# leochlon/aecf

Measured on AMD Instinct MI355X. Metric: fused samples/sec (fwd+bwd), higher is better.
Workload: dtype bf16; 1 GPU; c2: [B=65536 per GPU, M=3, d=512, 8 heads] mask_prob=0.15 train-mode curriculum masking, fwd+bwd; global_batch=65536, parallelism=dp1, world_size=1

## Files before the change

### aecf_amd/csrc/aecf_capi.hip

```cpp
#include <math.h>
#include <stdio.h>
#include <stdint.h>


#include "../../include/aecf_hip.h"
#include "aecf_kernels.h"

using namespace aecf;

namespace {

inline size_t align_up(size_t v, size_t a = 256) { return (v + a - 1) / a * a; }
inline int esize(int dtype) { return dtype == AECF_F32 ? 4 : 2; }
inline bool ws_frag_shape(int dtype, int E) { return dtype == AECF_BF16 && (E == 256 || E == 512 || E == 768 || E == 1024); }

struct FwdWs {
    size_t qs, a_f32, a_hi, a_lo, obuf, wv_frag, wo_frag, total;
};
FwdWs fwd_layout(const aecf_pool_desc* d) {
    FwdWs w;
    const size_t E = d->embed_dim, es = esize(d->dtype);
    size_t off = 0;
    w.qs = off;    off = align_up(off + E * 4);
    w.a_f32 = off; off = align_up(off + HPAD * E * 4);
// ... 399 lines not shown
    const BwdWs L = bwd_layout(d, hilo);
    if (a->workspace_bytes < L.total) return AECF_ERR_WORKSPACE;
    char* ws = (char*)a->workspace;
    const int E = d->embed_dim, H = d->num_heads, M = d->modalities, hd = E / H, es = esize(d->dtype);
    const int64_t B = d->batch;
    const PrepWs& P = L.prep;
    char* pb = a->saved_prep ? (char*)const_cast<void*>(a->saved_prep) : ws;
    float* qs = (float*)(pb + P.qs);
    float* a_f32 = (float*)(pb + P.a_f32);
    void* wvt = pb + P.wvt;
    void* wot = pb + P.wot;
    void* dobuf = do_ready ? const_cast<void*>(do_ready) : (void*)(ws + L.dobuf);
    float* dsbuf = (float*)(ws + L.dsbuf);
    float* u = (float*)(ws + L.u);
    const float scale = sqrtf(1.0f / (float)hd);
    const char* w_v = (const char*)a->w_in + (size_t)2 * E * E * es;

    void** ev = a->stage_events;
    mark(ev, 0, s);
    const bool frag = ws_frag_shape(d->dtype, E);
    FragJobs fj;
    if (!a->saved_prep) {
        if (frag) {
            fj.n = 2;
            fj.src[0] = w_v;      fj.dst[0] = pb + P.wvt_frag; fj.transposed[0] = 1;
            fj.src[1] = a->w_out; fj.dst[1] = pb + P.wot_frag; fj.transposed[1] = 1;
        }
        launch_prep_all(d->dtype, a->w_in, a->b_in, a->query, scale, qs, a_f32, pb + P.a_hi, pb + P.a_lo, w_v, wvt, a->w_out,
                        wot, E, H, fj, s);
    }
    mark(ev, 1, s);

    GemmNtArgs g;
    g.a = a->dy; g.w = wot; g.bias = nullptr; g.c = dobuf; g.probs = nullptr; g.R = B; g.N = E; g.K = E; g.lda = E;
    g.M = 1; g.H = H; g.hd = hd; g.pooled = 0; g.out_f32 = 0; g.v_out = nullptr;
    if (frag) g.w_frag = pb + P.wot_frag;
    if (hilo) g.c_lo = ws + L.do_lo;
    if (!do_ready) launch_gemm_nt(d->dtype, g, s);
    mark(ev, 2, s);

    GemmTnArgs t1;
    t1.lhs = a->dy; t1.rhs = a->saved_o; t1.probs = nullptr; t1.dsbuf = nullptr; t1.out = (float*)(ws + L.slab_o);
    t1.colsum = (float*)(ws + L.cs_o); t1.u = nullptr; t1.B = B; t1.M = 1; t1.E = E; t1.H = H; t1.hd = hd;
    t1.Ej = 0; t1.splits = L.splits; t1.rows_per_split = L.rows_per_split; t1.pooled = 0;
    t1.u_splits = 0; t1.u_rows_per_split = 0;
    if (hilo) {
        t1.rhs_lo = a->saved_o_lo;
        launch_gemm_tn_hilo(t1, s);
    } else {
        launch_gemm_tn(d->dtype, t1, s);
    }
    const int gt = a->grad_dtype == AECF_BF16 ? GRAD_BF16 : (a->grad_dtype == AECF_F16 ? GRAD_F16 : GRAD_F32);
    mark(ev, 3, s);

    BwdGArgs g2;
    g2.x = a->x; g2.dobuf = dobuf; g2.wvt = wvt; g2.probs = a->saved_probs; g2.d_attn_w = a->d_attn_w;
    g2.d_entropy = a->d_entropy; g2.attn_w = a->attn_w; g2.dsbuf = dsbuf; g2.a_f32 = a_f32; g2.dx = a->dx;
    g2.B = B; g2.M = M; g2.E = E; g2.H = H; g2.hd = hd; g2.log_M = (float)log((double)M);
    if (frag) g2.wvt_frag = pb + P.wvt_frag;
    int dsu_chunks = 0;
    if (hilo) g2.do_lo = ws + L.do_lo;
    const bool dsu = d->dtype == AECF_BF16 && dsu_ws_chunks(g2) > 0 && dsu_ws_chunks(g2) <= L.u_splits_cap &&
                     (!hilo || dsu_ws_takes_lo(g2));
    if (dsu)
        dsu_chunks = launch_dsu_ws(g2, (float*)(ws + L.u_slab), s);
    else if (!(!hilo && a->saved_v && launch_dscore_v(d->dtype, g2, a->saved_v, s)))
        launch_bwd_g(d->dtype, g2, false, s);
    mark(ev, 4, s);

    GemmTnArgs t2;
    t2.lhs = dobuf; t2.rhs = a->x; t2.probs = a->saved_probs; t2.dsbuf = dsbuf; t2.out = (float*)(ws + L.slab_v);
    t2.colsum = (float*)(ws + L.cs_v); t2.u = (float*)(ws + L.u_slab); t2.B = B; t2.M = M; t2.E = E; t2.H = H;
    t2.hd = hd; t2.Ej = 0; t2.splits = L.splits; t2.rows_per_split = L.rows_per_split; t2.pooled = 1;
    t2.u_splits = L.u_splits; t2.u_rows_per_split = L.u_rows_per_split;
    if (!dsu_chunks) {
        t2.parts = 2;
        launch_gemm_tn(d->dtype, t2, s);
    }
    mark(ev, 5, s);
    const bool dx_last = a->param_grads_event != nullptr;
    constexpr int DX_RESERVE_CUS = 16;
    if (dx_last) g2.cu_budget = 256 - DX_RESERVE_CUS;
    bool u_reduced = false;
    if (!dx_last) { g2.u_slab_in = (const float*)(ws + L.u_slab); g2.u_out = u; g2.u_nslab = dsu_chunks ? dsu_chunks : L.u_splits; }
    auto run_dx = [&]() {
        if (d->dtype == AECF_BF16 && launch_dx_ws(g2, s)) { u_reduced = g2.u_slab_in != nullptr; return; }
        launch_bwd_g(d->dtype, g2, true, s);
    };
// ... 633 lines not shown
```

### aecf_amd/csrc/aecf_gemm_ws.hip

```cpp
#include <stdlib.h>

#include "aecf_kernels.h"
#include "aecf_tile.h"

namespace aecf {

namespace {

enum { WS_PLAIN = 0, WS_VPROJ = 1, WS_VFLAT = 2 };

constexpr int WS_PF = 3, VPROJ_PF = 3, DX_PF = 3;

constexpr int ws_plain_bufs(int, int) { return 2; }

template <int KT, int NROWS, int KEYDIV>
__device__ __forceinline__ void ws_dma_rows(const char* __restrict__ src, unsigned int ld_bytes, int rows_valid, char* lds) {
    constexpr int CPR = 4 * KT;
    constexpr int TOTAL = NROWS * CPR;
    constexpr int NI = (TOTAL + 511) / 512;
    static_assert(TOTAL % 64 == 0, "whole wave-instructions");
    const int wbase = __builtin_amdgcn_readfirstlane((int)(threadIdx.x & ~63u));
#pragma unroll
    for (int i = 0; i < NI; ++i) {
        if (wbase + 512 * i < TOTAL) {
// ... 528 lines not shown
                for (int c = 0; c < CT; ++c) asm volatile("" : "+v"(acc[m][c]));
            __builtin_amdgcn_sched_barrier(0);
#pragma unroll
            for (int c = 0; c < CT; ++c) Pc[c] = Pn[c];
        }

        asm volatile("s_waitcnt vmcnt(0)" ::: "memory");
        if (o0 + 16 < o_end) park_stage(cur ^ 1);
        const int64_t b = o0 + r16;
        if (b < o_end) {
#pragma unroll
            for (int m = 0; m < M_; ++m) {
                float v[NV];
#pragma unroll
                for (int c = 0; c < CT; ++c)
#pragma unroll
                    for (int r = 0; r < 4; ++r) v[4 * c + r] = acc[m][c][r];
                store_cols<CT>(reinterpret_cast<unsigned short*>(p.dx) + (b * M_ + m) * E + ncol0 + NV * lg, v);
            }
        }
    }
}

template <int KT, int HK, int M_, bool HILO>
__global__ __launch_bounds__(512, 2) void dsu_ws_kernel(BwdGArgs p, float* __restrict__ u_slab, int rows_per_block, int nchunk) {
    using X = Tr<BF16>;
    constexpr int KJ = 8;
    constexpr int E = 32 * KT, JB = 32 * KJ, NCT = KT / 4;
    constexpr int HBL = KJ / HK;
    constexpr int ROWX = 2 * E, ROWD = 2 * JB;
    constexpr int XROWS = 16 * M_;
    constexpr int KU = (XROWS + 31) / 32;
    constexpr int ZROWS = (32 * KU - XROWS) > 0 ? 1 : 0;
    constexpr int PSTR = HBL * M_ * 16;
    constexpr int DSROW = 72;
    constexpr int XT = XROWS * ROWX, DT = 16 * ROWD;
    constexpr int NPART = 8;
    extern __shared__ __attribute__((aligned(16))) char smem[];
    char* xb = smem;
    char* zp = smem + 2 * XT;
    char* db = zp + ZROWS * ROWX;
    char* dbl = db + 2 * DT;
    float* part = reinterpret_cast<float*>(db + (HILO ? 4 : 2) * DT);
    unsigned short* dsh = reinterpret_cast<unsigned short*>(reinterpret_cast<char*>(part) + NPART * PSTR * 4);
    unsigned short* dsl = dsh + 16 * DSROW;

    const int lane = lane_id(), r16 = lane & 15, lg = lane >> 4;
    const int w = __builtin_amdgcn_readfirstlane(wave_id());
    const int H = p.H;
    unsigned int chunk_u, group_u;
    if (!xcd_tile(blockIdx.x, (unsigned)nchunk, (unsigned)(E / JB), chunk_u, group_u)) return;
    const int jbase = (int)group_u * JB, hbase = jbase / (32 * HK);
    const int ncol0 = 16 * NCT * w;
    const int64_t o_beg = (int64_t)chunk_u * rows_per_block;
    const int64_t o_end = (o_beg + rows_per_block) < p.B ? (o_beg + rows_per_block) : p.B;
    if (o_beg >= o_end) return;

    const char* dsrc = reinterpret_cast<const char*>(p.dobuf) + (int64_t)jbase * 2;
    const char* xsrc = reinterpret_cast<const char*>(p.x);
    const char* dlsrc = HILO ? reinterpret_cast<const char*>(p.do_lo) + (int64_t)jbase * 2 : dsrc;
    auto issue = [&](int64_t o0, int buf) {
        const int ov = (int)((o_end - o0) < 16 ? (o_end - o0) : 16);
        ws_dma_rows_asm<KT, 16 * M_, M_>(xsrc + o0 * M_ * (int64_t)ROWX, (unsigned)ROWX, ov * M_, xb + buf * XT);
        ws_dma_rows_asm<KJ, 16, 1>(dsrc + o0 * (int64_t)ROWX, (unsigned)ROWX, ov, db + buf * DT);
        if (HILO) ws_dma_rows_asm<KJ, 16, 1>(dlsrc + o0 * (int64_t)ROWX, (unsigned)ROWX, ov, dbl + buf * DT);
    };
    for (int i = threadIdx.x; i < ZROWS * ROWX / 16; i += 512) reinterpret_cast<u32x4*>(zp)[i] = u32x4{0u, 0u, 0u, 0u};
    for (int i = threadIdx.x; i < 2 * 16 * DSROW / 2; i += 512) reinterpret_cast<unsigned int*>(dsh)[i] = 0u;
    issue(o_beg, 0);

    const unsigned short* wsrc = reinterpret_cast<const unsigned short*>(p.wvt);
    u32x4 wreg[KJ][NCT];
    static_assert(NCT % 2 == 0, "tile pairs");
#pragma unroll
    for (int ct = 0; ct < NCT; ++ct) {
        const int krow = ncol0 + 32 * (ct >> 1) + 8 * (r16 >> 2) + 4 * (ct & 1) + (r16 & 3);
        const unsigned short* wr = wsrc + (int64_t)krow * E + jbase + 8 * lg;
#pragma unroll
        for (int ks = 0; ks < KJ; ++ks) wreg[ks][ct] = *reinterpret_cast<const u32x4*>(wr + 32 * ks);
    }
    int daddr[4];
#pragma unroll
    for (int v = 0; v < 4; ++v) daddr[v] = r16 * ROWD + ((((4 * v) + lg) ^ r16) << 4);
    const int xaddr0 = r16 * M_ * ROWX + ((((ncol0 >> 3) + lg) ^ r16) << 4);
    const int q = r16 >> 2, pp = r16 & 3;
    int ua[KU][2];
    bool uz[KU][2];
#pragma unroll
    for (int ks = 0; ks < KU; ++ks) {
#pragma unroll
        for (int hh = 0; hh < 2; ++hh) {
            const int D = 4 * ks + 2 * hh + (lg >> 1);
            uz[ks][hh] = D >= 2 * M_;
            const int m = D >> 1, b = 2 * (4 * (lg & 1) + q) + (D & 1);
            const int key = uz[ks][hh] ? 0 : b;
            const int ch = ((ncol0 >> 3) + (pp >> 1)) ^ key;
            ua[ks][hh] = (uz[ks][hh] ? (int)(zp - smem) : (b * M_ + m) * ROWX) + (ch << 4) + 8 * (pp & 1);
        }
    }
    auto kslot = [&](int b, int m) -> int {
        const int D = 2 * m + (b & 1), j = b >> 1;
        return 32 * (D >> 2) + 8 * (2 * (D & 1) + (j >> 2)) + 4 * ((D >> 1) & 1) + (j & 3);
    };

    const int ds_s = lane & 15, ds_hh = w, ds_m = lg;
    const float invH = 1.0f / (float)H;
    auto load_stats = [&](int64_t o0, float& pmv, float& dwb) {
        int64_t b = o0 + ds_s;
        b = b < o_end ? b : o_end - 1;
        const float* pp_ = p.probs + (b * H + hbase + ds_hh) * M_ + (ds_m < M_ ? ds_m : 0);
        const float* dw_ = p.d_attn_w ? p.d_attn_w + b * M_ + (ds_m < M_ ? ds_m : 0) : pp_;
        if (w < HBL) {
            asm volatile("global_load_dword %0, %1, off" : "=v"(pmv) : "v"(pp_) : "memory");
            asm volatile("global_load_dword %0, %1, off" : "=v"(dwb) : "v"(dw_) : "memory");
        }
    };

    f32x4 uacc[NCT];
#pragma unroll
    for (int ct = 0; ct < NCT; ++ct) uacc[ct] = f32x4{0.f, 0.f, 0.f, 0.f};
    float pmv = 0.f, dwb = 0.f, pmv_n = 0.f, dwb_n = 0.f;
#pragma unroll
    for (int ks = 0; ks < KJ; ++ks)
#pragma unroll
        for (int ct = 0; ct < NCT; ++ct) asm volatile("" : "+v"(wreg[ks][ct]));
    load_stats(o_beg, pmv, dwb);

    asm volatile("s_waitcnt vmcnt(0)" ::: "memory");
    asm volatile("s_waitcnt lgkmcnt(0)" ::: "memory");
    int cur = 0;
    for (int64_t o0 = o_beg; o0 < o_end; o0 += 16, cur ^= 1) {
        __builtin_amdgcn_s_barrier();
        if (o0 + 16 < o_end) {
            issue(o0 + 16, cur ^ 1);
            load_stats(o0 + 16, pmv_n, dwb_n);
        }
        const char* tb = db + cur * DT;
        constexpr int HG = HBL % 2 == 0 ? 2 : 1;
        int xa[NCT];
#pragma unroll
        for (int ct = 0; ct < NCT; ++ct) xa[ct] = cur * XT + (xaddr0 ^ (64 * (ct >> 1)));
        float* pw = part + w * PSTR + r16;
#pragma unroll
        for (int h0 = 0; h0 < HBL; h0 += HG) {
            f32x4 P[HG][NCT];
#pragma unroll
            for (int g = 0; g < HG; ++g) {
#pragma unroll
                for (int ct = 0; ct < NCT; ++ct) P[g][ct] = f32x4{0.f, 0.f, 0.f, 0.f};
#pragma unroll
                for (int kl = 0; kl < HK; ++kl) {
                    const int ks = (h0 + g) * HK + kl;
                    const u32x4 bf = *reinterpret_cast<const u32x4*>(tb + daddr[ks & 3] + (ks >> 2) * 256);
#pragma unroll
                    for (int ct = 0; ct < NCT; ++ct) P[g][ct] = X::mma(wreg[ks][ct], bf, P[g][ct]);
                    if (HILO) {
                        const u32x4 bl = *reinterpret_cast<const u32x4*>(dbl + cur * DT + daddr[ks & 3] + (ks >> 2) * 256);
#pragma unroll
                        for (int ct = 0; ct < NCT; ++ct) P[g][ct] = X::mma(wreg[ks][ct], bl, P[g][ct]);
                    }
                }
            }
#pragma unroll
            for (int m = 0; m < M_; ++m) {
                float a[HG];
#pragma unroll
                for (int g = 0; g < HG; ++g) a[g] = 0.f;
#pragma unroll
                for (int c2 = 0; c2 < NCT / 2; ++c2) {
                    const u32x4 xv = *reinterpret_cast<const u32x4*>(xb + xa[2 * c2] + m * ROWX);
                    float xf[8];
#pragma unroll
                    for (int i = 0; i < 4; ++i) {
                        xf[2 * i] = __uint_as_float(xv[i] << 16);
                        xf[2 * i + 1] = __uint_as_float(xv[i] & 0xffff0000u);
                    }
#pragma unroll
                    for (int g = 0; g < HG; ++g)
#pragma unroll
                        for (int i = 0; i < 8; ++i) a[g] = fmaf(P[g][2 * c2 + (i >> 2)][i & 3], xf[i], a[g]);
                }
                const unsigned int u0 = __float_as_uint(a[0]), u1 = __float_as_uint(a[HG - 1]);
                const auto r1 = __builtin_amdgcn_permlane16_swap(u0, u1, false, false);
                const unsigned int us = __float_as_uint(__uint_as_float(r1[0]) + __uint_as_float(r1[1]));
                const auto r2 = __builtin_amdgcn_permlane32_swap(us, us, false, false);
                pw[((h0 + (HG == 2 ? (lg & 1) : 0)) * M_ + m) * 16] = __uint_as_float(r2[0]) + __uint_as_float(r2[1]);
            }
        }
        asm volatile("s_waitcnt lgkmcnt(0)" ::: "memory");
        __builtin_amdgcn_s_barrier();
        asm volatile("" : "+v"(pmv), "+v"(dwb));
        if (w < HBL) {
            float da = 0.f;
            if (ds_m < M_) {
                const float* pr = part + (ds_hh * M_ + ds_m) * 16 + ds_s;
#pragma unroll
                for (int i = 0; i < NPART; ++i) da += pr[i * PSTR];
            }
            float dw = p.d_attn_w ? dwb : 0.f;
            if (p.d_entropy && ds_m < M_) {
                int64_t be = o0 + ds_s;
                be = be < o_end ? be : o_end - 1;
                float hsum = 0.f;
#pragma unroll
                for (int m = 0; m < M_; ++m) hsum -= xlogx(p.attn_w[be * M_ + m]);
                const bool live = (hsum >= 0.f) && (hsum <= p.log_M);
                dw += live ? -(logf(p.attn_w[be * M_ + ds_m]) + 1.0f) * p.d_entropy[be] : 0.f;
            }
            const float dp = da + dw * invH;
            const float dot = reduce_lg((ds_m < M_) ? pmv * dp : 0.f);
            const int64_t b = o0 + ds_s;
            if (ds_m < M_) {
                const float d = (b < o_end) ? pmv * (dp - dot) : 0.f;
                if (b < o_end) p.dsbuf[(b * H + hbase + ds_hh) * M_ + ds_m] = d;
                const unsigned short hi = X::from_f32(d);
                dsh[ds_hh * DSROW + kslot(ds_s, ds_m)] = hi;
                dsl[ds_hh * DSROW + kslot(ds_s, ds_m)] = X::from_f32(d - X::to_f32(hi));
            }
        }
        asm volatile("s_waitcnt lgkmcnt(0)" ::: "memory");
        __builtin_amdgcn_s_barrier();
#pragma unroll
        for (int ks = 0; ks < KU; ++ks) {
            const u32x4 bh = *reinterpret_cast<const u32x4*>(reinterpret_cast<const char*>(dsh) + (r16 * DSROW + 32 * ks + 8 * lg) * 2);
            const u32x4 bl = *reinterpret_cast<const u32x4*>(reinterpret_cast<const char*>(dsl) + (r16 * DSROW + 32 * ks + 8 * lg) * 2);
#pragma unroll
            for (int ct = 0; ct < NCT; ++ct) {
                const u32x4 af = tr_frag16(smem, (uz[ks][0] ? 0 : cur * XT) + (ua[ks][0] ^ (32 * ct)),
                                           (uz[ks][1] ? 0 : cur * XT) + (ua[ks][1] ^ (32 * ct)));
                uacc[ct] = X::mma(af, bh, uacc[ct]);
                uacc[ct] = X::mma(af, bl, uacc[ct]);
            }
        }
        asm volatile("s_waitcnt vmcnt(0)" ::: "memory");
        asm volatile("" : "+v"(pmv_n), "+v"(dwb_n));
        pmv = pmv_n; dwb = dwb_n;
    }
    if (r16 < HBL) {
#pragma unroll
        for (int ct = 0; ct < NCT; ++ct)
            *reinterpret_cast<f32x4*>(u_slab + ((int64_t)chunk_u * H + hbase + r16) * E + ncol0 + 16 * ct + 4 * lg) = uacc[ct];
    }
}


static size_t dsu_ws_smem(int E, int M, int hd, bool lo) {
    constexpr int JB = 256;
    const int xrows = 16 * M, zrows = (32 * ((xrows + 31) / 32) - xrows) > 0 ? 1 : 0, hbl = JB / hd;
    return (size_t)(2 * xrows + zrows) * 2 * E + (size_t)(lo ? 4 : 2) * 16 * 2 * JB + (size_t)8 * (16 * hbl * M) * 4 +
           (size_t)2 * 16 * 72 * 2;
}

template <int KT, int HK, int M_>
int launch_dsu_t(const BwdGArgs& a, float* u_slab, hipStream_t s) {
    constexpr int E = 32 * KT, JB = 256;
    const bool hilo = a.do_lo && dsu_ws_takes_lo(a);
    const size_t smem = dsu_ws_smem(E, M_, a.hd, hilo);
    const int groups = E / JB;
    int64_t chunks = 256 / groups;
    if (chunks < 1) chunks = 1;
    int64_t rpb = (a.B + chunks - 1) / chunks;
    rpb = (rpb + 15) / 16 * 16;
    const int64_t nchunk = (a.B + rpb - 1) / rpb;
    dim3 grid(xcd_grid((unsigned)nchunk, (unsigned)groups)), block(512);
    if constexpr (!(E == 512 && M_ == 4)) {
        if (hilo) {
            auto kern = dsu_ws_kernel<KT, HK, M_, true>;
            (void)hipFuncSetAttribute(reinterpret_cast<const void*>(kern), hipFuncAttributeMaxDynamicSharedMemorySize, (int)smem);
            kern<<<grid, block, smem, s>>>(a, u_slab, (int)rpb, (int)nchunk);
            return (int)nchunk;
        }
    }
    auto kern = dsu_ws_kernel<KT, HK, M_, false>;
    (void)hipFuncSetAttribute(reinterpret_cast<const void*>(kern), hipFuncAttributeMaxDynamicSharedMemorySize, (int)smem);
    kern<<<grid, block, smem, s>>>(a, u_slab, (int)rpb, (int)nchunk);
    return (int)nchunk;
}

template <int KT, int HK, int M_>
void launch_dx2(const BwdGArgs& a, hipStream_t s) {
    constexpr int K = 32 * KT;
    constexpr int CT = KT <= 16 ? 2 : 1;
    constexpr int KX = (3 * (KT / HK) + 31) / 32;
    const size_t smem = (size_t)2 * 16 * 2 * K + (size_t)2 * 16 * (((KT / HK) * M_) | 1) * sizeof(float) + (size_t)2 * 16 * M_ * (64 * KX + 16);
    const int groups = a.E / (128 * CT);
    int64_t chunks = (a.cu_budget > 0 ? a.cu_budget : 256) / groups;
    if (chunks < 1) chunks = 1;
    int64_t rpb = (a.B + chunks - 1) / chunks;
    rpb = (rpb + 15) / 16 * 16;
    const int64_t nchunk = (a.B + rpb - 1) / rpb;
    dim3 grid(xcd_grid((unsigned)nchunk, (unsigned)groups)), block(512);
    auto kern = dx_ws2_kernel<KT, HK, M_, CT>;
    if (smem > 64 * 1024)
        (void)hipFuncSetAttribute(reinterpret_cast<const void*>(kern), hipFuncAttributeMaxDynamicSharedMemorySize, (int)smem);
    kern<<<grid, block, smem, s>>>(a, (int)rpb, (int)nchunk);
}

template <int KT, int HK>
void launch_dx2_m(const BwdGArgs& a, hipStream_t s) {
    switch (a.M) {
        case 1: launch_dx2<KT, HK, 1>(a, s); break;
// ... 301 lines not shown
    return a.lda == a.K;
}

void launch_gemm_ws(const GemmNtArgs& a, hipStream_t s) {
    if (ws_vproj_flat(a)) {
        GemmNtArgs f = a;
        f.R = a.R * a.M;
        f.lda = a.K;
        launch_kt<WS_VFLAT, 4, false>(f, s);
        return;
    }
    if (a.pooled & 1) {
        switch (a.M) {
            case 1: if (a.g_ahi) launch_kt<WS_VPROJ, 1, true>(a, s); else launch_kt<WS_VPROJ, 1, false>(a, s); break;
            case 2: if (a.g_ahi) launch_kt<WS_VPROJ, 2, true>(a, s); else launch_kt<WS_VPROJ, 2, false>(a, s); break;
            case 3: if (a.g_ahi) launch_kt<WS_VPROJ, 3, true>(a, s); else launch_kt<WS_VPROJ, 3, false>(a, s); break;
            default: launch_kt<WS_VPROJ, 4, false>(a, s); break;
        }
    } else {
        launch_kt<WS_PLAIN, 1, false>(a, s);
    }
}

int dsu_ws_chunks(const BwdGArgs& a) {
    if (a.M < 1 || a.M > 4 || a.hd % 32 != 0 || a.E != a.H * a.hd) return 0;
    if (a.E != 256 && a.E != 512) return 0;
    const int jb = 256;
    if (jb % a.hd != 0) return 0;
    const int hk = a.hd / 32;
    if (hk != 1 && hk != 2 && hk != 4 && hk != 8) return 0;
    if (dsu_ws_smem(a.E, a.M, a.hd, false) > 160 * 1024) return 0;
    const int groups = a.E / jb;
    int64_t chunks = 256 / groups;
    int64_t rpb = (a.B + chunks - 1) / chunks;
    rpb = (rpb + 15) / 16 * 16;
    return (int)((a.B + rpb - 1) / rpb);
}

bool dsu_ws_takes_lo(const BwdGArgs& a) {
    return dsu_ws_chunks(a) > 0 && dsu_ws_smem(a.E, a.M, a.hd, true) <= 160 * 1024;
}

template <int KT, int HK>
static int launch_dsu_m(const BwdGArgs& a, float* u_slab, hipStream_t s) {
    switch (a.M) {
        case 1: return launch_dsu_t<KT, HK, 1>(a, u_slab, s);
        case 2: return launch_dsu_t<KT, HK, 2>(a, u_slab, s);
        case 3: return launch_dsu_t<KT, HK, 3>(a, u_slab, s);
        default: return launch_dsu_t<KT, HK, 4>(a, u_slab, s);
    }
}

int launch_dsu_ws(const BwdGArgs& a, float* u_slab, hipStream_t s) {
    if (dsu_ws_chunks(a) == 0) return 0;
    const int hk = a.hd / 32;
#define DSU_CASE(KT_)                                                   \
    switch (hk) {                                                       \
        case 1: return launch_dsu_m<KT_, 1>(a, u_slab, s);              \
        case 2: return launch_dsu_m<KT_, 2>(a, u_slab, s);              \
        case 4: return launch_dsu_m<KT_, 4>(a, u_slab, s);              \
        default: return launch_dsu_m<KT_, 8>(a, u_slab, s);             \
    }
    if (a.E == 256) { DSU_CASE(8) }
    DSU_CASE(16)
#undef DSU_CASE
}

bool launch_dx_ws(const BwdGArgs& a, hipStream_t s) {
    if (a.M < 1 || a.M > 4) return false;
    if (a.hd % 32 != 0 || a.E != a.H * a.hd || 16 * a.H * a.M > 1024) return false;
    switch (a.E) {
        case 256: return launch_dx2_hk<8>(a, s);
        case 512: return launch_dx2_hk<16>(a, s);
        case 768: return launch_dx2_hk<24>(a, s);
        case 1024: return launch_dx2_hk<32>(a, s);
        default: return false;
    }
}

}
```

### aecf_amd/csrc/aecf_kernels.h

```cpp
#pragma once
#include <hip/hip_runtime.h>
#include <stdint.h>

#include "aecf_common.h"

namespace aecf {

constexpr int HPAD = 16;

void launch_prep_qs(int dtype, const void* w_in, const void* b_in, const void* query, float* qs, int E, float scale,
                    hipStream_t s);
void launch_prep_amat(int dtype, const void* w_in, const float* qs, float* a_f32, void* a_hi, void* a_lo, int E, int H,
                      hipStream_t s);
void launch_transpose(int dtype, const void* src, void* dst, int E, hipStream_t s);
struct FragJobs {
    int n = 0;
    const void* src[4] = {nullptr, nullptr, nullptr, nullptr};
    void* dst[4] = {nullptr, nullptr, nullptr, nullptr};
    int transposed[4] = {0, 0, 0, 0};
};
void launch_prep_all(int dtype, const void* w_in, const void* b_in, const void* query, float scale, float* qs, float* a_f32,
                     void* a_hi, void* a_lo, const void* t_src0, void* t_dst0, const void* t_src1, void* t_dst1, int E,
                     int H, const FragJobs& fj, hipStream_t s);

// ... 57 lines not shown
    const void* dobuf;
    const void* wvt;
    const float* probs;
    const float* d_attn_w;
    const float* d_entropy;
    const float* attn_w;
    float* dsbuf;
    const float* a_f32;
    void* dx;
    int64_t B;
    int M, E, H, hd;
    float log_M;
    const void* wvt_frag = nullptr;
    int cu_budget = 0;
    const float* u_slab_in = nullptr;
    float* u_out = nullptr;
    int u_nslab = 0;
    const void* do_lo = nullptr;
};
void launch_bwd_g(int dtype, const BwdGArgs& a, bool dx, hipStream_t s);
bool launch_dscore_v(int dtype, const BwdGArgs& a, const void* saved_v, hipStream_t s);
bool launch_dx_ws(const BwdGArgs& a, hipStream_t s);
int dsu_ws_chunks(const BwdGArgs& a);
int launch_dsu_ws(const BwdGArgs& a, float* u_slab, hipStream_t s);
bool dsu_ws_takes_lo(const BwdGArgs& a);

struct GemmTnArgs {
    const void* lhs;
    const void* rhs;
    const float* probs;
    const float* dsbuf;
    float* out;
    float* colsum;
    float* u;
    int64_t B;
    int M, E, H, hd;
    int Ej;
    int splits;
    int64_t rows_per_split;
    int u_splits;
    int64_t u_rows_per_split;
    int pooled;
    int parts = 0;
    DqpJob dq;
    const void* lhs_lo = nullptr;
    const void* rhs_lo = nullptr;
};
// ... 123 lines not shown
```

Before: 123.1 million samples/s.

## Reassociate dscore backward to project x through Wv instead of dO through WvT

Replaces the fused dscore+u kernel with a new one that computes v = x·Wv per modality (Wv held in registers, loaded from a newly prepared non-transposed fragment copy) and dots it with dO directly. The old path staged dO tiles into LDS and multiplied by WvT to get P before dotting with x. The change removes dO LDS staging and the per-head P accumulators, cutting LDS footprint and MMA work per row block. In exchange it needs an extra weight-fragment prep job, and the associativity change alters rounding.

```diff
diff --git a/aecf_amd/csrc/aecf_capi.hip b/aecf_amd/csrc/aecf_capi.hip
--- a/aecf_amd/csrc/aecf_capi.hip
+++ b/aecf_amd/csrc/aecf_capi.hip
@@ -445,9 +445,10 @@
     FragJobs fj;
     if (!a->saved_prep) {
         if (frag) {
-            fj.n = 2;
+            fj.n = 3;
             fj.src[0] = w_v;      fj.dst[0] = pb + P.wvt_frag; fj.transposed[0] = 1;
             fj.src[1] = a->w_out; fj.dst[1] = pb + P.wot_frag; fj.transposed[1] = 1;
+            fj.src[2] = w_v;      fj.dst[2] = pb + P.wv_frag;  fj.transposed[2] = 0;
         }
         launch_prep_all(d->dtype, a->w_in, a->b_in, a->query, scale, qs, a_f32, pb + P.a_hi, pb + P.a_lo, w_v, wvt, a->w_out,
                         wot, E, H, fj, s);
@@ -486,7 +487,7 @@
     const bool dsu = d->dtype == AECF_BF16 && dsu_ws_chunks(g2) > 0 && dsu_ws_chunks(g2) <= L.u_splits_cap &&
                      (!hilo || dsu_ws_takes_lo(g2));
     if (dsu)
-        dsu_chunks = launch_dsu_ws(g2, (float*)(ws + L.u_slab), s);
+        dsu_chunks = launch_dsu_ws(g2, w_v, frag ? pb + P.wv_frag : nullptr, (float*)(ws + L.u_slab), s);
     else if (!(!hilo && a->saved_v && launch_dscore_v(d->dtype, g2, a->saved_v, s)))
         launch_bwd_g(d->dtype, g2, false, s);
     mark(ev, 4, s);
diff --git a/aecf_amd/csrc/aecf_dsv_ws.hip b/aecf_amd/csrc/aecf_dsv_ws.hip
--- /dev/null
+++ b/aecf_amd/csrc/aecf_dsv_ws.hip
@@ -0,0 +1,314 @@
+#include "aecf_kernels.h"
+#include "aecf_tile.h"
+
+namespace aecf {
+
+namespace {
+
+constexpr int DSV_PF = 3;
+
+template <int KT, int HK, int M_, bool HILO>
+__global__ __launch_bounds__(512, 2) void dsv_ws_kernel(BwdGArgs p, const void* __restrict__ wv, const void* __restrict__ wv_frag,
+                                                         float* __restrict__ u_slab, int rows_per_block, int nchunk) {
+    using X = Tr<BF16>;
+    constexpr int E = 32 * KT, JB = 256, NCT = KT / 4;
+    constexpr int HBL = 8 / HK;
+    constexpr int ROWX = 2 * E;
+    constexpr int XROWS = 16 * M_;
+    constexpr int KU = (XROWS + 31) / 32;
+    constexpr int ZROWS = (32 * KU - XROWS) > 0 ? 1 : 0;
+    constexpr int PSTR = M_ * 16;
+    constexpr int DSROW = 72;
+    constexpr int XT = XROWS * ROWX;
+    extern __shared__ __attribute__((aligned(16))) char smem[];
+    char* xb = smem;
+    char* zp = smem + 2 * XT;
+    float* part = reinterpret_cast<float*>(zp + ZROWS * ROWX);
+    unsigned short* dsh = reinterpret_cast<unsigned short*>(reinterpret_cast<char*>(part) + 8 * PSTR * 4);
+    unsigned short* dsl = dsh + 16 * DSROW;
+
+    const int lane = lane_id(), r16 = lane & 15, lg = lane >> 4;
+    const int w = __builtin_amdgcn_readfirstlane(wave_id());
+    const int H = p.H;
+    unsigned int chunk_u, group_u;
+    if (!xcd_tile(blockIdx.x, (unsigned)nchunk, (unsigned)(E / JB), chunk_u, group_u)) return;
+    const int jbase = (int)group_u * JB, hbase = jbase / (32 * HK);
+    const int jcol0 = jbase + 32 * w;
+    const int ncol0 = 16 * NCT * w;
+    const int64_t o_beg = (int64_t)chunk_u * rows_per_block;
+    const int64_t o_end = (o_beg + rows_per_block) < p.B ? (o_beg + rows_per_block) : p.B;
+    if (o_beg >= o_end) return;
+
+    const char* xsrc = reinterpret_cast<const char*>(p.x);
+    auto issue = [&](int64_t o0, int buf) {
+        const int ov = (int)((o_end - o0) < 16 ? (o_end - o0) : 16);
+        ws_dma_rows_asm<KT, 16 * M_, M_>(xsrc + o0 * M_ * (int64_t)ROWX, (unsigned)ROWX, ov * M_, xb + buf * XT);
+    };
+    for (int i = threadIdx.x; i < ZROWS * ROWX / 16; i += 512) reinterpret_cast<u32x4*>(zp)[i] = u32x4{0u, 0u, 0u, 0u};
+    for (int i = threadIdx.x; i < 2 * 16 * DSROW / 2; i += 512) reinterpret_cast<unsigned int*>(dsh)[i] = 0u;
+    issue(o_beg, 0);
+
+    u32x4 wreg[KT][2];
+#pragma unroll
+    for (int c = 0; c < 2; ++c) {
+        const int n = jcol0 + 8 * (r16 >> 2) + 4 * c + (r16 & 3);
+        const unsigned short* wr = reinterpret_cast<const unsigned short*>(wv) + (int64_t)n * E + 8 * lg;
+        const u32x4* wf = reinterpret_cast<const u32x4*>(wv_frag) + ((int64_t)((jcol0 / 32) * 2 + c) * KT) * 64 + lane;
+#pragma unroll
+        for (int ks = 0; ks < KT; ++ks) wreg[ks][c] = wv_frag ? wf[ks * 64] : *reinterpret_cast<const u32x4*>(wr + 32 * ks);
+    }
+    int xaddr[4];
+#pragma unroll
+    for (int v = 0; v < 4; ++v) xaddr[v] = r16 * M_ * ROWX + ((((4 * v) + lg) ^ r16) << 4);
+
+    const int q = r16 >> 2, pp = r16 & 3;
+    int ua[KU][2];
+    bool uz[KU][2];
+#pragma unroll
+    for (int ks = 0; ks < KU; ++ks) {
+#pragma unroll
+        for (int hh = 0; hh < 2; ++hh) {
+            const int D = 4 * ks + 2 * hh + (lg >> 1);
+            uz[ks][hh] = D >= 2 * M_;
+            const int m = D >> 1, b = 2 * (4 * (lg & 1) + q) + (D & 1);
+            const int key = uz[ks][hh] ? 0 : b;
+            const int ch = ((ncol0 >> 3) + (pp >> 1)) ^ key;
+            ua[ks][hh] = (uz[ks][hh] ? (int)(zp - smem) : (b * M_ + m) * ROWX) + (ch << 4) + 8 * (pp & 1);
+        }
+    }
+    auto kslot = [&](int b, int m) -> int {
+        const int D = 2 * m + (b & 1), j = b >> 1;
+        return 32 * (D >> 2) + 8 * (2 * (D & 1) + (j >> 2)) + 4 * ((D >> 1) & 1) + (j & 3);
+    };
+
+    const int ds_s = lane & 15, ds_hh = w, ds_m = lg;
+    const float invH = 1.0f / (float)H;
+    auto load_stats = [&](int64_t o0, float& pmv, float& dwb) {
+        int64_t b = o0 + ds_s;
+        b = b < o_end ? b : o_end - 1;
+        const float* pp_ = p.probs + (b * H + hbase + (ds_hh < HBL ? ds_hh : 0)) * M_ + (ds_m < M_ ? ds_m : 0);
+        const float* dw_ = p.d_attn_w ? p.d_attn_w + b * M_ + (ds_m < M_ ? ds_m : 0) : pp_;
+        if (w < HBL) {
+            asm volatile("global_load_dword %0, %1, off" : "=v"(pmv) : "v"(pp_) : "memory");
+            asm volatile("global_load_dword %0, %1, off" : "=v"(dwb) : "v"(dw_) : "memory");
+        }
+    };
+    const unsigned short* dsrc = reinterpret_cast<const unsigned short*>(p.dobuf) + jcol0 + 8 * lg;
+    const unsigned short* dlsrc = HILO ? reinterpret_cast<const unsigned short*>(p.do_lo) + jcol0 + 8 * lg : dsrc;
+    auto load_do = [&](int64_t o0, u32x4& dh, u32x4& dl) {
+        int64_t b = o0 + r16;
+        b = b < o_end ? b : o_end - 1;
+        const unsigned short* ph = dsrc + b * E;
+        asm volatile("global_load_dwordx4 %0, %1, off" : "=v"(dh) : "v"(ph) : "memory");
+        if (HILO) {
+            const unsigned short* pl = dlsrc + b * E;
+            asm volatile("global_load_dwordx4 %0, %1, off" : "=v"(dl) : "v"(pl) : "memory");
+        }
+    };
+
+    f32x4 uacc[NCT];
+#pragma unroll
+    for (int ct = 0; ct < NCT; ++ct) uacc[ct] = f32x4{0.f, 0.f, 0.f, 0.f};
+    float pmv = 0.f, dwb = 0.f, pmv_n = 0.f, dwb_n = 0.f;
+    u32x4 dh = u32x4{0u, 0u, 0u, 0u}, dl = dh, dh_n = dh, dl_n = dh;
+#pragma unroll
+    for (int ks = 0; ks < KT; ++ks)
+#pragma unroll
+        for (int c = 0; c < 2; ++c) asm volatile("" : "+v"(wreg[ks][c]));
+    load_stats(o_beg, pmv, dwb);
+    load_do(o_beg, dh, dl);
+
+    asm volatile("s_waitcnt vmcnt(0)" ::: "memory");
+    asm volatile("s_waitcnt lgkmcnt(0)" ::: "memory");
+    int cur = 0;
+    for (int64_t o0 = o_beg; o0 < o_end; o0 += 16, cur ^= 1) {
+        asm volatile("" : "+v"(dh));
+        if (HILO) asm volatile("" : "+v"(dl));
+        float dof[8];
+#pragma unroll
+        for (int i = 0; i < 4; ++i) {
+            dof[2 * i] = __uint_as_float(dh[i] << 16);
+            dof[2 * i + 1] = __uint_as_float(dh[i] & 0xffff0000u);
+            if (HILO) {
+                dof[2 * i] += __uint_as_float(dl[i] << 16);
+                dof[2 * i + 1] += __uint_as_float(dl[i] & 0xffff0000u);
+            }
+        }
+        __builtin_amdgcn_s_barrier();
+        if (o0 + 16 < o_end) {
+            issue(o0 + 16, cur ^ 1);
+            load_stats(o0 + 16, pmv_n, dwb_n);
+            load_do(o0 + 16, dh_n, dl_n);
+        }
+        constexpr int NIT = M_ * KT, PF = DSV_PF;
+        const char* tb = xb + cur * XT;
+        auto rd = [&](int i) -> u32x4 {
+            const int ks = i % KT, m = i / KT;
+            return *reinterpret_cast<const u32x4*>(tb + xaddr[ks & 3] + m * ROWX + (ks >> 2) * 256);
+        };
+        f32x4 acc[2];
+#pragma unroll
+        for (int c = 0; c < 2; ++c) acc[c] = f32x4{0.f, 0.f, 0.f, 0.f};
+        float a[M_];
+        u32x4 xf[PF + 1];
+#pragma unroll
+        for (int i = 0; i < PF; ++i) xf[i] = rd(i);
+        __builtin_amdgcn_sched_group_barrier(0x100, PF, 0);
+#pragma unroll
+        for (int i = 0; i < NIT; ++i) {
+            if (i + PF < NIT) xf[(i + PF) % (PF + 1)] = rd(i + PF);
+            const int ks = i % KT;
+#pragma unroll
+            for (int c = 0; c < 2; ++c) acc[c] = X::mma(wreg[ks][c], xf[i % (PF + 1)], acc[c]);
+            __builtin_amdgcn_sched_group_barrier(0x100, 1, 0);
+            __builtin_amdgcn_sched_group_barrier(0x008, 2, 0);
+            if (ks == KT - 1) {
+                float s = 0.f;
+#pragma unroll
+                for (int c = 0; c < 2; ++c)
+#pragma unroll
+                    for (int r = 0; r < 4; ++r) s = fmaf(acc[c][r], dof[4 * c + r], s);
+                a[i / KT] = s;
+#pragma unroll
+                for (int c = 0; c < 2; ++c) acc[c] = f32x4{0.f, 0.f, 0.f, 0.f};
+            }
+        }
+        float* pw = part + w * PSTR + r16;
+#pragma unroll
+        for (int m = 0; m < M_; ++m) {
+            const unsigned int u0 = __float_as_uint(a[m]);
+            const auto r1 = __builtin_amdgcn_permlane16_swap(u0, u0, false, false);
+            const unsigned int us = __float_as_uint(__uint_as_float(r1[0]) + __uint_as_float(r1[1]));
+            const auto r2 = __builtin_amdgcn_permlane32_swap(us, us, false, false);
+            pw[m * 16] = __uint_as_float(r2[0]) + __uint_as_float(r2[1]);
+        }
+        asm volatile("s_waitcnt lgkmcnt(0)" ::: "memory");
+        __builtin_amdgcn_s_barrier();
+        asm volatile("" : "+v"(pmv), "+v"(dwb));
+        if (w < HBL) {
+            float da = 0.f;
+            if (ds_m < M_) {
+                const float* pr = part + ds_hh * HK * PSTR + ds_m * 16 + ds_s;
+#pragma unroll
+                for (int i = 0; i < HK; ++i) da += pr[i * PSTR];
+            }
+            float dw = p.d_attn_w ? dwb : 0.f;
+            if (p.d_entropy && ds_m < M_) {
+                int64_t be = o0 + ds_s;
+                be = be < o_end ? be : o_end - 1;
+                float hsum = 0.f;
+#pragma unroll
+                for (int m = 0; m < M_; ++m) hsum -= xlogx(p.attn_w[be * M_ + m]);
+                const bool live = (hsum >= 0.f) && (hsum <= p.log_M);
+                dw += live ? -(logf(p.attn_w[be * M_ + ds_m]) + 1.0f) * p.d_entropy[be] : 0.f;
+            }
+            const float dp = da + dw * invH;
+            const float dot = reduce_lg((ds_m < M_) ? pmv * dp : 0.f);
+            const int64_t b = o0 + ds_s;
+            if (ds_m < M_) {
+                const float d = (b < o_end) ? pmv * (dp - dot) : 0.f;
+                if (b < o_end) p.dsbuf[(b * H + hbase + ds_hh) * M_ + ds_m] = d;
+                const unsigned short hi = X::from_f32(d);
+                dsh[ds_hh * DSROW + kslot(ds_s, ds_m)] = hi;
+                dsl[ds_hh * DSROW + kslot(ds_s, ds_m)] = X::from_f32(d - X::to_f32(hi));
+            }
+        }
+        asm volatile("s_waitcnt lgkmcnt(0)" ::: "memory");
+        __builtin_amdgcn_s_barrier();
+#pragma unroll
+        for (int ks = 0; ks < KU; ++ks) {
+            const u32x4 bh = *reinterpret_cast<const u32x4*>(reinterpret_cast<const char*>(dsh) + (r16 * DSROW + 32 * ks + 8 * lg) * 2);
+            const u32x4 bl = *reinterpret_cast<const u32x4*>(reinterpret_cast<const char*>(dsl) + (r16 * DSROW + 32 * ks + 8 * lg) * 2);
+#pragma unroll
+            for (int ct = 0; ct < NCT; ++ct) {
+                const u32x4 af = tr_frag16(smem, (uz[ks][0] ? 0 : cur * XT) + (ua[ks][0] ^ (32 * ct)),
+                                           (uz[ks][1] ? 0 : cur * XT) + (ua[ks][1] ^ (32 * ct)));
+                uacc[ct] = X::mma(af, bh, uacc[ct]);
+                uacc[ct] = X::mma(af, bl, uacc[ct]);
+            }
+        }
+        asm volatile("s_waitcnt vmcnt(0)" ::: "memory");
+        asm volatile("" : "+v"(pmv_n), "+v"(dwb_n), "+v"(dh_n));
+        pmv = pmv_n; dwb = dwb_n; dh = dh_n;
+        if (HILO) { asm volatile("" : "+v"(dl_n)); dl = dl_n; }
+    }
+    if (r16 < HBL) {
+#pragma unroll
+        for (int ct = 0; ct < NCT; ++ct)
+            *reinterpret_cast<f32x4*>(u_slab + ((int64_t)chunk_u * H + hbase + r16) * E + ncol0 + 16 * ct + 4 * lg) = uacc[ct];
+    }
+}
+
+constexpr size_t dsv_ws_smem(int E, int M) {
+    const int xrows = 16 * M, zrows = (32 * ((xrows + 31) / 32) - xrows) > 0 ? 1 : 0;
+    return (size_t)(2 * xrows + zrows) * 2 * E + (size_t)8 * 16 * M * 4 + (size_t)2 * 16 * 72 * 2;
+}
+
+template <int KT, int HK, int M_>
+int launch_dsv_t(const BwdGArgs& a, const void* wv, const void* wv_frag, float* u_slab, hipStream_t s) {
+    constexpr int E = 32 * KT, JB = 256;
+    constexpr size_t smem = dsv_ws_smem(E, M_);
+    static_assert(smem <= 160 * 1024, "LDS");
+    const int groups = E / JB;
+    int64_t chunks = 256 / groups;
+    int64_t rpb = (a.B + chunks - 1) / chunks;
+    rpb = (rpb + 15) / 16 * 16;
+    const int64_t nchunk = (a.B + rpb - 1) / rpb;
+    dim3 grid(xcd_grid((unsigned)nchunk, (unsigned)groups)), block(512);
+    if constexpr (!(E == 512 && M_ == 4)) {
+        if (a.do_lo) {
+            auto kern = dsv_ws_kernel<KT, HK, M_, true>;
+            (void)hipFuncSetAttribute(reinterpret_cast<const void*>(kern), hipFuncAttributeMaxDynamicSharedMemorySize, (int)smem);
+            kern<<<grid, block, smem, s>>>(a, wv, wv_frag, u_slab, (int)rpb, (int)nchunk);
+            return (int)nchunk;
+        }
+    }
+    auto kern = dsv_ws_kernel<KT, HK, M_, false>;
+    (void)hipFuncSetAttribute(reinterpret_cast<const void*>(kern), hipFuncAttributeMaxDynamicSharedMemorySize, (int)smem);
+    kern<<<grid, block, smem, s>>>(a, wv, wv_frag, u_slab, (int)rpb, (int)nchunk);
+    return (int)nchunk;
+}
+
+template <int KT, int HK>
+int launch_dsv_m(const BwdGArgs& a, const void* wv, const void* wv_frag, float* u_slab, hipStream_t s) {
+    switch (a.M) {
+        case 1: return launch_dsv_t<KT, HK, 1>(a, wv, wv_frag, u_slab, s);
+        case 2: return launch_dsv_t<KT, HK, 2>(a, wv, wv_frag, u_slab, s);
+        case 3: return launch_dsv_t<KT, HK, 3>(a, wv, wv_frag, u_slab, s);
+        default: return launch_dsv_t<KT, HK, 4>(a, wv, wv_frag, u_slab, s);
+    }
+}
+
+}
+
+int dsu_ws_chunks(const BwdGArgs& a) {
+    if (a.M < 1 || a.M > 4 || a.hd % 32 != 0 || a.E != a.H * a.hd) return 0;
+    if (a.E != 256 && a.E != 512) return 0;
+    const int hk = a.hd / 32;
+    if (hk != 1 && hk != 2 && hk != 4 && hk != 8) return 0;
+    if (dsv_ws_smem(a.E, a.M) > 160 * 1024) return 0;
+    const int groups = a.E / 256;
+    int64_t chunks = 256 / groups;
+    int64_t rpb = (a.B + chunks - 1) / chunks;
+    rpb = (rpb + 15) / 16 * 16;
+    return (int)((a.B + rpb - 1) / rpb);
+}
+
+bool dsu_ws_takes_lo(const BwdGArgs& a) { return dsu_ws_chunks(a) > 0 && !(a.E == 512 && a.M == 4); }
+
+int launch_dsu_ws(const BwdGArgs& a, const void* wv, const void* wv_frag, float* u_slab, hipStream_t s) {
+    if (dsu_ws_chunks(a) == 0) return 0;
+    const int hk = a.hd / 32;
+#define DSV_CASE(KT_)                                                           \
+    switch (hk) {                                                               \
+        case 1: return launch_dsv_m<KT_, 1>(a, wv, wv_frag, u_slab, s);         \
+        case 2: return launch_dsv_m<KT_, 2>(a, wv, wv_frag, u_slab, s);         \
+        case 4: return launch_dsv_m<KT_, 4>(a, wv, wv_frag, u_slab, s);         \
+        default: return launch_dsv_m<KT_, 8>(a, wv, wv_frag, u_slab, s);        \
+    }
+    if (a.E == 256) { DSV_CASE(8) }
+    DSV_CASE(16)
+#undef DSV_CASE
+}
+
+}
diff --git a/aecf_amd/csrc/aecf_gemm_ws.hip b/aecf_amd/csrc/aecf_gemm_ws.hip
--- a/aecf_amd/csrc/aecf_gemm_ws.hip
+++ b/aecf_amd/csrc/aecf_gemm_ws.hip
@@ -574,261 +574,6 @@
     }
 }
 
-template <int KT, int HK, int M_, bool HILO>
-__global__ __launch_bounds__(512, 2) void dsu_ws_kernel(BwdGArgs p, float* __restrict__ u_slab, int rows_per_block, int nchunk) {
-    using X = Tr<BF16>;
-    constexpr int KJ = 8;
-    constexpr int E = 32 * KT, JB = 32 * KJ, NCT = KT / 4;
-    constexpr int HBL = KJ / HK;
-    constexpr int ROWX = 2 * E, ROWD = 2 * JB;
-    constexpr int XROWS = 16 * M_;
-    constexpr int KU = (XROWS + 31) / 32;
-    constexpr int ZROWS = (32 * KU - XROWS) > 0 ? 1 : 0;
-    constexpr int PSTR = HBL * M_ * 16;
-    constexpr int DSROW = 72;
-    constexpr int XT = XROWS * ROWX, DT = 16 * ROWD;
-    constexpr int NPART = 8;
-    extern __shared__ __attribute__((aligned(16))) char smem[];
-    char* xb = smem;
-    char* zp = smem + 2 * XT;
-    char* db = zp + ZROWS * ROWX;
-    char* dbl = db + 2 * DT;
-    float* part = reinterpret_cast<float*>(db + (HILO ? 4 : 2) * DT);
-    unsigned short* dsh = reinterpret_cast<unsigned short*>(reinterpret_cast<char*>(part) + NPART * PSTR * 4);
-    unsigned short* dsl = dsh + 16 * DSROW;
-
-    const int lane = lane_id(), r16 = lane & 15, lg = lane >> 4;
-    const int w = __builtin_amdgcn_readfirstlane(wave_id());
-    const int H = p.H;
-    unsigned int chunk_u, group_u;
-    if (!xcd_tile(blockIdx.x, (unsigned)nchunk, (unsigned)(E / JB), chunk_u, group_u)) return;
-    const int jbase = (int)group_u * JB, hbase = jbase / (32 * HK);
-    const int ncol0 = 16 * NCT * w;
-    const int64_t o_beg = (int64_t)chunk_u * rows_per_block;
-    const int64_t o_end = (o_beg + rows_per_block) < p.B ? (o_beg + rows_per_block) : p.B;
-    if (o_beg >= o_end) return;
-
-    const char* dsrc = reinterpret_cast<const char*>(p.dobuf) + (int64_t)jbase * 2;
-    const char* xsrc = reinterpret_cast<const char*>(p.x);
-    const char* dlsrc = HILO ? reinterpret_cast<const char*>(p.do_lo) + (int64_t)jbase * 2 : dsrc;
-    auto issue = [&](int64_t o0, int buf) {
-        const int ov = (int)((o_end - o0) < 16 ? (o_end - o0) : 16);
-        ws_dma_rows_asm<KT, 16 * M_, M_>(xsrc + o0 * M_ * (int64_t)ROWX, (unsigned)ROWX, ov * M_, xb + buf * XT);
-        ws_dma_rows_asm<KJ, 16, 1>(dsrc + o0 * (int64_t)ROWX, (unsigned)ROWX, ov, db + buf * DT);
-        if (HILO) ws_dma_rows_asm<KJ, 16, 1>(dlsrc + o0 * (int64_t)ROWX, (unsigned)ROWX, ov, dbl + buf * DT);
-    };
-    for (int i = threadIdx.x; i < ZROWS * ROWX / 16; i += 512) reinterpret_cast<u32x4*>(zp)[i] = u32x4{0u, 0u, 0u, 0u};
-    for (int i = threadIdx.x; i < 2 * 16 * DSROW / 2; i += 512) reinterpret_cast<unsigned int*>(dsh)[i] = 0u;
-    issue(o_beg, 0);
-
-    const unsigned short* wsrc = reinterpret_cast<const unsigned short*>(p.wvt);
-    u32x4 wreg[KJ][NCT];
-    static_assert(NCT % 2 == 0, "tile pairs");
-#pragma unroll
-    for (int ct = 0; ct < NCT; ++ct) {
-        const int krow = ncol0 + 32 * (ct >> 1) + 8 * (r16 >> 2) + 4 * (ct & 1) + (r16 & 3);
-        const unsigned short* wr = wsrc + (int64_t)krow * E + jbase + 8 * lg;
-#pragma unroll
-        for (int ks = 0; ks < KJ; ++ks) wreg[ks][ct] = *reinterpret_cast<const u32x4*>(wr + 32 * ks);
-    }
-    int daddr[4];
-#pragma unroll
-    for (int v = 0; v < 4; ++v) daddr[v] = r16 * ROWD + ((((4 * v) + lg) ^ r16) << 4);
-    const int xaddr0 = r16 * M_ * ROWX + ((((ncol0 >> 3) + lg) ^ r16) << 4);
-    const int q = r16 >> 2, pp = r16 & 3;
-    int ua[KU][2];
-    bool uz[KU][2];
-#pragma unroll
-    for (int ks = 0; ks < KU; ++ks) {
-#pragma unroll
-        for (int hh = 0; hh < 2; ++hh) {
-            const int D = 4 * ks + 2 * hh + (lg >> 1);
-            uz[ks][hh] = D >= 2 * M_;
-            const int m = D >> 1, b = 2 * (4 * (lg & 1) + q) + (D & 1);
-            const int key = uz[ks][hh] ? 0 : b;
-            const int ch = ((ncol0 >> 3) + (pp >> 1)) ^ key;
-            ua[ks][hh] = (uz[ks][hh] ? (int)(zp - smem) : (b * M_ + m) * ROWX) + (ch << 4) + 8 * (pp & 1);
-        }
-    }
-    auto kslot = [&](int b, int m) -> int {
-        const int D = 2 * m + (b & 1), j = b >> 1;
-        return 32 * (D >> 2) + 8 * (2 * (D & 1) + (j >> 2)) + 4 * ((D >> 1) & 1) + (j & 3);
-    };
-
-    const int ds_s = lane & 15, ds_hh = w, ds_m = lg;
-    const float invH = 1.0f / (float)H;
-    auto load_stats = [&](int64_t o0, float& pmv, float& dwb) {
-        int64_t b = o0 + ds_s;
-        b = b < o_end ? b : o_end - 1;
-        const float* pp_ = p.probs + (b * H + hbase + ds_hh) * M_ + (ds_m < M_ ? ds_m : 0);
-        const float* dw_ = p.d_attn_w ? p.d_attn_w + b * M_ + (ds_m < M_ ? ds_m : 0) : pp_;
-        if (w < HBL) {
-            asm volatile("global_load_dword %0, %1, off" : "=v"(pmv) : "v"(pp_) : "memory");
-            asm volatile("global_load_dword %0, %1, off" : "=v"(dwb) : "v"(dw_) : "memory");
-        }
-    };
-
-    f32x4 uacc[NCT];
-#pragma unroll
-    for (int ct = 0; ct < NCT; ++ct) uacc[ct] = f32x4{0.f, 0.f, 0.f, 0.f};
-    float pmv = 0.f, dwb = 0.f, pmv_n = 0.f, dwb_n = 0.f;
-#pragma unroll
-    for (int ks = 0; ks < KJ; ++ks)
-#pragma unroll
-        for (int ct = 0; ct < NCT; ++ct) asm volatile("" : "+v"(wreg[ks][ct]));
-    load_stats(o_beg, pmv, dwb);
-
-    asm volatile("s_waitcnt vmcnt(0)" ::: "memory");
-    asm volatile("s_waitcnt lgkmcnt(0)" ::: "memory");
-    int cur = 0;
-    for (int64_t o0 = o_beg; o0 < o_end; o0 += 16, cur ^= 1) {
-        __builtin_amdgcn_s_barrier();
-        if (o0 + 16 < o_end) {
-            issue(o0 + 16, cur ^ 1);
-            load_stats(o0 + 16, pmv_n, dwb_n);
-        }
-        const char* tb = db + cur * DT;
-        constexpr int HG = HBL % 2 == 0 ? 2 : 1;
-        int xa[NCT];
-#pragma unroll
-        for (int ct = 0; ct < NCT; ++ct) xa[ct] = cur * XT + (xaddr0 ^ (64 * (ct >> 1)));
-        float* pw = part + w * PSTR + r16;
-#pragma unroll
-        for (int h0 = 0; h0 < HBL; h0 += HG) {
-            f32x4 P[HG][NCT];
-#pragma unroll
-            for (int g = 0; g < HG; ++g) {
-#pragma unroll
-                for (int ct = 0; ct < NCT; ++ct) P[g][ct] = f32x4{0.f, 0.f, 0.f, 0.f};
-#pragma unroll
-                for (int kl = 0; kl < HK; ++kl) {
-                    const int ks = (h0 + g) * HK + kl;
-                    const u32x4 bf = *reinterpret_cast<const u32x4*>(tb + daddr[ks & 3] + (ks >> 2) * 256);
-#pragma unroll
-                    for (int ct = 0; ct < NCT; ++ct) P[g][ct] = X::mma(wreg[ks][ct], bf, P[g][ct]);
-                    if (HILO) {
-                        const u32x4 bl = *reinterpret_cast<const u32x4*>(dbl + cur * DT + daddr[ks & 3] + (ks >> 2) * 256);
-#pragma unroll
-                        for (int ct = 0; ct < NCT; ++ct) P[g][ct] = X::mma(wreg[ks][ct], bl, P[g][ct]);
-                    }
-                }
-            }
-#pragma unroll
-            for (int m = 0; m < M_; ++m) {
-                float a[HG];
-#pragma unroll
-                for (int g = 0; g < HG; ++g) a[g] = 0.f;
-#pragma unroll
-                for (int c2 = 0; c2 < NCT / 2; ++c2) {
-                    const u32x4 xv = *reinterpret_cast<const u32x4*>(xb + xa[2 * c2] + m * ROWX);
-                    float xf[8];
-#pragma unroll
-                    for (int i = 0; i < 4; ++i) {
-                        xf[2 * i] = __uint_as_float(xv[i] << 16);
-                        xf[2 * i + 1] = __uint_as_float(xv[i] & 0xffff0000u);
-                    }
-#pragma unroll
-                    for (int g = 0; g < HG; ++g)
-#pragma unroll
-                        for (int i = 0; i < 8; ++i) a[g] = fmaf(P[g][2 * c2 + (i >> 2)][i & 3], xf[i], a[g]);
-                }
-                const unsigned int u0 = __float_as_uint(a[0]), u1 = __float_as_uint(a[HG - 1]);
-                const auto r1 = __builtin_amdgcn_permlane16_swap(u0, u1, false, false);
-                const unsigned int us = __float_as_uint(__uint_as_float(r1[0]) + __uint_as_float(r1[1]));
-                const auto r2 = __builtin_amdgcn_permlane32_swap(us, us, false, false);
-                pw[((h0 + (HG == 2 ? (lg & 1) : 0)) * M_ + m) * 16] = __uint_as_float(r2[0]) + __uint_as_float(r2[1]);
-            }
-        }
-        asm volatile("s_waitcnt lgkmcnt(0)" ::: "memory");
-        __builtin_amdgcn_s_barrier();
-        asm volatile("" : "+v"(pmv), "+v"(dwb));
-        if (w < HBL) {
-            float da = 0.f;
-            if (ds_m < M_) {
-                const float* pr = part + (ds_hh * M_ + ds_m) * 16 + ds_s;
-#pragma unroll
-                for (int i = 0; i < NPART; ++i) da += pr[i * PSTR];
-            }
-            float dw = p.d_attn_w ? dwb : 0.f;
-            if (p.d_entropy && ds_m < M_) {
-                int64_t be = o0 + ds_s;
-                be = be < o_end ? be : o_end - 1;
-                float hsum = 0.f;
-#pragma unroll
-                for (int m = 0; m < M_; ++m) hsum -= xlogx(p.attn_w[be * M_ + m]);
-                const bool live = (hsum >= 0.f) && (hsum <= p.log_M);
-                dw += live ? -(logf(p.attn_w[be * M_ + ds_m]) + 1.0f) * p.d_entropy[be] : 0.f;
-            }
-            const float dp = da + dw * invH;
-            const float dot = reduce_lg((ds_m < M_) ? pmv * dp : 0.f);
-            const int64_t b = o0 + ds_s;
-            if (ds_m < M_) {
-                const float d = (b < o_end) ? pmv * (dp - dot) : 0.f;
-                if (b < o_end) p.dsbuf[(b * H + hbase + ds_hh) * M_ + ds_m] = d;
-                const unsigned short hi = X::from_f32(d);
-                dsh[ds_hh * DSROW + kslot(ds_s, ds_m)] = hi;
-                dsl[ds_hh * DSROW + kslot(ds_s, ds_m)] = X::from_f32(d - X::to_f32(hi));
-            }
-        }
-        asm volatile("s_waitcnt lgkmcnt(0)" ::: "memory");
-        __builtin_amdgcn_s_barrier();
-#pragma unroll
-        for (int ks = 0; ks < KU; ++ks) {
-            const u32x4 bh = *reinterpret_cast<const u32x4*>(reinterpret_cast<const char*>(dsh) + (r16 * DSROW + 32 * ks + 8 * lg) * 2);
-            const u32x4 bl = *reinterpret_cast<const u32x4*>(reinterpret_cast<const char*>(dsl) + (r16 * DSROW + 32 * ks + 8 * lg) * 2);
-#pragma unroll
-            for (int ct = 0; ct < NCT; ++ct) {
-                const u32x4 af = tr_frag16(smem, (uz[ks][0] ? 0 : cur * XT) + (ua[ks][0] ^ (32 * ct)),
-                                           (uz[ks][1] ? 0 : cur * XT) + (ua[ks][1] ^ (32 * ct)));
-                uacc[ct] = X::mma(af, bh, uacc[ct]);
-                uacc[ct] = X::mma(af, bl, uacc[ct]);
-            }
-        }
-        asm volatile("s_waitcnt vmcnt(0)" ::: "memory");
-        asm volatile("" : "+v"(pmv_n), "+v"(dwb_n));
-        pmv = pmv_n; dwb = dwb_n;
-    }
-    if (r16 < HBL) {
-#pragma unroll
-        for (int ct = 0; ct < NCT; ++ct)
-            *reinterpret_cast<f32x4*>(u_slab + ((int64_t)chunk_u * H + hbase + r16) * E + ncol0 + 16 * ct + 4 * lg) = uacc[ct];
-    }
-}
-
-
-static size_t dsu_ws_smem(int E, int M, int hd, bool lo) {
-    constexpr int JB = 256;
-    const int xrows = 16 * M, zrows = (32 * ((xrows + 31) / 32) - xrows) > 0 ? 1 : 0, hbl = JB / hd;
-    return (size_t)(2 * xrows + zrows) * 2 * E + (size_t)(lo ? 4 : 2) * 16 * 2 * JB + (size_t)8 * (16 * hbl * M) * 4 +
-           (size_t)2 * 16 * 72 * 2;
-}
-
-template <int KT, int HK, int M_>
-int launch_dsu_t(const BwdGArgs& a, float* u_slab, hipStream_t s) {
-    constexpr int E = 32 * KT, JB = 256;
-    const bool hilo = a.do_lo && dsu_ws_takes_lo(a);
-    const size_t smem = dsu_ws_smem(E, M_, a.hd, hilo);
-    const int groups = E / JB;
-    int64_t chunks = 256 / groups;
-    if (chunks < 1) chunks = 1;
-    int64_t rpb = (a.B + chunks - 1) / chunks;
-    rpb = (rpb + 15) / 16 * 16;
-    const int64_t nchunk = (a.B + rpb - 1) / rpb;
-    dim3 grid(xcd_grid((unsigned)nchunk, (unsigned)groups)), block(512);
-    if constexpr (!(E == 512 && M_ == 4)) {
-        if (hilo) {
-            auto kern = dsu_ws_kernel<KT, HK, M_, true>;
-            (void)hipFuncSetAttribute(reinterpret_cast<const void*>(kern), hipFuncAttributeMaxDynamicSharedMemorySize, (int)smem);
-            kern<<<grid, block, smem, s>>>(a, u_slab, (int)rpb, (int)nchunk);
-            return (int)nchunk;
-        }
-    }
-    auto kern = dsu_ws_kernel<KT, HK, M_, false>;
-    (void)hipFuncSetAttribute(reinterpret_cast<const void*>(kern), hipFuncAttributeMaxDynamicSharedMemorySize, (int)smem);
-    kern<<<grid, block, smem, s>>>(a, u_slab, (int)rpb, (int)nchunk);
-    return (int)nchunk;
-}
-
 template <int KT, int HK, int M_>
 void launch_dx2(const BwdGArgs& a, hipStream_t s) {
     constexpr int K = 32 * KT;
@@ -1176,50 +921,6 @@
     }
 }
 
-int dsu_ws_chunks(const BwdGArgs& a) {
-    if (a.M < 1 || a.M > 4 || a.hd % 32 != 0 || a.E != a.H * a.hd) return 0;
-    if (a.E != 256 && a.E != 512) return 0;
-    const int jb = 256;
-    if (jb % a.hd != 0) return 0;
-    const int hk = a.hd / 32;
-    if (hk != 1 && hk != 2 && hk != 4 && hk != 8) return 0;
-    if (dsu_ws_smem(a.E, a.M, a.hd, false) > 160 * 1024) return 0;
-    const int groups = a.E / jb;
-    int64_t chunks = 256 / groups;
-    int64_t rpb = (a.B + chunks - 1) / chunks;
-    rpb = (rpb + 15) / 16 * 16;
-    return (int)((a.B + rpb - 1) / rpb);
-}
-
-bool dsu_ws_takes_lo(const BwdGArgs& a) {
-    return dsu_ws_chunks(a) > 0 && dsu_ws_smem(a.E, a.M, a.hd, true) <= 160 * 1024;
-}
-
-template <int KT, int HK>
-static int launch_dsu_m(const BwdGArgs& a, float* u_slab, hipStream_t s) {
-    switch (a.M) {
-        case 1: return launch_dsu_t<KT, HK, 1>(a, u_slab, s);
-        case 2: return launch_dsu_t<KT, HK, 2>(a, u_slab, s);
-        case 3: return launch_dsu_t<KT, HK, 3>(a, u_slab, s);
-        default: return launch_dsu_t<KT, HK, 4>(a, u_slab, s);
-    }
-}
-
-int launch_dsu_ws(const BwdGArgs& a, float* u_slab, hipStream_t s) {
-    if (dsu_ws_chunks(a) == 0) return 0;
-    const int hk = a.hd / 32;
-#define DSU_CASE(KT_)                                                   \
-    switch (hk) {                                                       \
-        case 1: return launch_dsu_m<KT_, 1>(a, u_slab, s);              \
-        case 2: return launch_dsu_m<KT_, 2>(a, u_slab, s);              \
-        case 4: return launch_dsu_m<KT_, 4>(a, u_slab, s);              \
-        default: return launch_dsu_m<KT_, 8>(a, u_slab, s);             \
-    }
-    if (a.E == 256) { DSU_CASE(8) }
-    DSU_CASE(16)
-#undef DSU_CASE
-}
-
 bool launch_dx_ws(const BwdGArgs& a, hipStream_t s) {
     if (a.M < 1 || a.M > 4) return false;
     if (a.hd % 32 != 0 || a.E != a.H * a.hd || 16 * a.H * a.M > 1024) return false;
diff --git a/aecf_amd/csrc/aecf_kernels.h b/aecf_amd/csrc/aecf_kernels.h
--- a/aecf_amd/csrc/aecf_kernels.h
+++ b/aecf_amd/csrc/aecf_kernels.h
@@ -103,7 +103,7 @@
 bool launch_dscore_v(int dtype, const BwdGArgs& a, const void* saved_v, hipStream_t s);
 bool launch_dx_ws(const BwdGArgs& a, hipStream_t s);
 int dsu_ws_chunks(const BwdGArgs& a);
-int launch_dsu_ws(const BwdGArgs& a, float* u_slab, hipStream_t s);
+int launch_dsu_ws(const BwdGArgs& a, const void* wv, const void* wv_frag, float* u_slab, hipStream_t s);
 bool dsu_ws_takes_lo(const BwdGArgs& a);
 
 struct GemmTnArgs {
```

Result: no change. 123.7 million samples/s (median of 5 runs) (+0.5%).
